# hedgepigdaniel/video-annotator

Measured on AMD Instinct MI355X. Metric: stabilized frames/sec at 4K NV12, 1/2/4/8 GPU; remap % HBM roofline, higher is better.
Workload: dtype u8 pixels / f32 map / f64 rotations

## Files before the change

video-annotator_amd/csrc/vstab_track.hip:

```cpp
#include <algorithm>
#include <climits>

#include <hip/hip_ext.h>

#include "vstab_internal.hpp"
#include "vstab_track.hpp"

namespace vstab {

__device__ __forceinline__ int reflect101(int i, int n) {
    if (n == 1) return 0;
    while (i < 0 || i >= n) i = i < 0 ? -i : 2 * n - 2 - i;
    return i;
}

__device__ __forceinline__ uint32_t load4_reflect_row(const uint8_t *__restrict__ row, int w, int gx, bool vec_ok) {
    if (vec_ok && gx >= 0 && gx + 4 <= w) return *reinterpret_cast<const uint32_t *>(row + gx);
    uint32_t v = 0;
#pragma unroll
    for (int i = 0; i < 4; i++) v |= (uint32_t)row[reflect101(gx + i, w)] << (8 * i);
    return v;
}

__device__ __forceinline__ uint32_t load4_reflect(const uint8_t *__restrict__ src, uint32_t pitch, int w, int h, int gx,
// ... 51 lines not shown
                d[j][0] = p[0], d[j][1] = p[1], d[j][2] = p[2], d[j][3] = p[3];
            }
        }
    } else {
#pragma unroll
        for (int q = 0; q < 4; q++) {
            const int gx = sx0 + 4 * q;
            if (vec_ok && gx >= 0 && gx + 4 <= sw) {
#pragma unroll
                for (int j = 0; j < 5; j++) d[j][q] = *reinterpret_cast<const uint32_t *>(row[j] + gx);
            } else {
                int col[4];
#pragma unroll
                for (int i = 0; i < 4; i++) col[i] = NEAR ? min(abs(gx + i), 2 * sw - 2 - abs(gx + i)) : reflect101(gx + i, sw);
#pragma unroll
                for (int j = 0; j < 5; j++)
                    d[j][q] = (uint32_t)row[j][col[0]] | ((uint32_t)row[j][col[1]] << 8) | ((uint32_t)row[j][col[2]] << 16) | ((uint32_t)row[j][col[3]] << 24);
            }
        }
    }
    if (COPY) {
#pragma unroll
        for (int jj = 2; jj <= 3; jj++) {
            const int r = 2 * y + jj - 2;
            if (r >= sh) break;
            uint8_t *o = cp + (uint32_t)r * cpitch + (uint32_t)(2 * x0);
            if (!EDGE) {
                *reinterpret_cast<uint2 *>(o) = make_uint2(d[jj][1], d[jj][2]);
            } else {
#pragma unroll
                for (int b = 0; b < 8; b++)
                    if (2 * x0 + b < sw) o[b] = (uint8_t)((b < 4 ? d[jj][1] : d[jj][2]) >> (8 * (b & 3)));
            }
        }
    }
    return pyr_down_dot4x4(d);
}

template <bool EDGE, bool NEAR, bool COPY = false>
__device__ __forceinline__ void pyr_down_group(const uint8_t *__restrict__ src, uint32_t spitch, int sw, int sh, uint8_t *__restrict__ dst, size_t dpitch,
                                               int dw, int x0, int y, bool vec_ok, uint8_t *__restrict__ cp = nullptr, uint32_t cpitch = 0) {
    const uint32_t out = pyr_down_group4<EDGE, NEAR, COPY>(src, spitch, sw, sh, x0, y, vec_ok, cp, cpitch);
    uint8_t *o = dst + (size_t)((uint32_t)y * (uint32_t)dpitch) + x0;
    if (!EDGE) {
        *reinterpret_cast<uint32_t *>(o) = out;
    } else {
        for (int c = 0; c < 4 && x0 + c < dw; c++) o[c] = (uint8_t)(out >> (8 * c));
    }
}

__global__ void __launch_bounds__(256) k_pyr_down(const uint8_t *__restrict__ src, size_t spitch, int sw, int sh,
                                                  uint8_t *__restrict__ dst, size_t dpitch, int dw, int dh, int vec_ok, int g_lo, int g_hi,
                                                  int nbx, int nb_edge, int n_groups, int near) {
    if ((int)blockIdx.x >= nb_edge) {
        const int b = blockIdx.x - nb_edge, by = b / nbx, bx = b - by * nbx;
        const int g = g_lo + bx * 64 + (threadIdx.x & 63), y = by * 4 + (threadIdx.x >> 6);
        if (g >= g_hi || y >= dh) return;
        pyr_down_group<false, true>(src, (uint32_t)spitch, sw, sh, dst, dpitch, dw, 4 * g, y, true);
    } else {
        const int n_edge = n_groups - (g_hi - g_lo);
        const int e = blockIdx.x * 256 + threadIdx.x;
        const int y = e / n_edge, i = e - y * n_edge;
        if (y >= dh) return;
        const int g = i < g_lo ? i : g_hi + (i - g_lo);
        if (near)
            pyr_down_group<true, true>(src, (uint32_t)spitch, sw, sh, dst, dpitch, dw, 4 * g, y, vec_ok != 0);
        else
            pyr_down_group<true, false>(src, (uint32_t)spitch, sw, sh, dst, dpitch, dw, 4 * g, y, vec_ok != 0);
    }
}

__global__ void __launch_bounds__(256) k_pack_pyr(const uint8_t *__restrict__ src, uint32_t spitch, int sw, int sh, uint8_t *__restrict__ dst, uint32_t dpitch,
                                                  int dw, int dh, int vec_ok, int g_lo, int g_hi, int nbx, int nb_edge, int n_groups, int near, int nb_pyr,
                                                  const uint8_t *__restrict__ uv, uint32_t uvpitch, uint8_t *__restrict__ ring, uint32_t rpitch, int uv_vec) {
    if ((int)blockIdx.x >= nb_pyr) {
        uint8_t *cdst = ring + (uint32_t)sh * rpitch;
        const int rows = sh / 2;
        if (uv_vec) {
            const int vecs = sw / 16;
            for (int e = ((int)blockIdx.x - nb_pyr) * 256 + threadIdx.x; e < rows * vecs; e += ((int)gridDim.x - nb_pyr) * 256) {
                const int r = e / vecs, c = e - r * vecs;
                reinterpret_cast<uint4 *>(cdst + (uint32_t)r * rpitch)[c] = reinterpret_cast<const uint4 *>(uv + (uint32_t)r * uvpitch)[c];
            }
        } else {
            for (int e = ((int)blockIdx.x - nb_pyr) * 256 + threadIdx.x; e < rows * sw; e += ((int)gridDim.x - nb_pyr) * 256) {
                const int r = e / sw, c = e - r * sw;
                cdst[(uint32_t)r * rpitch + c] = uv[(uint32_t)r * uvpitch + c];
            }
        }
        return;
    }
    if ((int)blockIdx.x >= nb_edge) {
        const int b = blockIdx.x - nb_edge, by = b / nbx, bx = b - by * nbx;
        const int g = g_lo + bx * 64 + (threadIdx.x & 63), y = by * 4 + (threadIdx.x >> 6);
        if (g >= g_hi || y >= dh) return;
        pyr_down_group<false, true, true>(src, spitch, sw, sh, dst, dpitch, dw, 4 * g, y, true, ring, rpitch);
    } else {
        const int n_edge = n_groups - (g_hi - g_lo);
        const int e = blockIdx.x * 256 + threadIdx.x;
        const int y = e / n_edge, i = e - y * n_edge;
        if (y >= dh) return;
        const int g = i < g_lo ? i : g_hi + (i - g_lo);
        if (near)
            pyr_down_group<true, true, true>(src, spitch, sw, sh, dst, dpitch, dw, 4 * g, y, vec_ok != 0, ring, rpitch);
        else
            pyr_down_group<true, false, true>(src, spitch, sw, sh, dst, dpitch, dw, 4 * g, y, vec_ok != 0, ring, rpitch);
    }
}

constexpr int P2_TW = 16, P2_TH = 10;
constexpr int P2_MG = (2 * P2_TW + 5 + 3) / 4, P2_MW = 4 * P2_MG;
constexpr int P2_MH = 2 * P2_TH + 3;
constexpr int P2_ITEMS = P2_MG * P2_MH, P2_ROUNDS = (P2_ITEMS + 255) / 256;
static_assert(P2_TW % 4 == 0 && 2 * P2_TW + 5 <= P2_MW, "the region holds the taps of the tile's last output");

template <bool NEAR>
__device__ __forceinline__ void pyr_down_x2_tile(const uint8_t *__restrict__ src, uint32_t spitch, int sw, int sh, uint8_t *__restrict__ mid, uint32_t mpitch, int mw,
                                                 int mh, uint8_t *__restrict__ dst, uint32_t dpitch, int dw, int dh, bool vec_ok, bool dst_vec_ok,
                                                 uint8_t (&smid)[P2_MH][P2_MW]) {
    const int tid = threadIdx.x;
    const int x0 = blockIdx.x * P2_TW, y0 = blockIdx.y * P2_TH;
    const int mx0 = 2 * x0 - 4, my0 = 2 * y0 - 2;
    const bool interior = vec_ok && mx0 >= 2 && my0 >= 1 && mx0 + P2_MW <= mw && my0 + P2_MH <= mh && 2 * (mx0 + P2_MW) + 4 <= sw && 2 * (my0 + P2_MH) + 1 <= sh;
    if (interior) {
        uint32_t d[P2_ROUNDS][5][4];
#pragma unroll
        for (int k = 0; k < P2_ROUNDS; k++) {
            const int it = min(tid + 256 * k, P2_ITEMS - 1);
            const int ry = it / P2_MG, g = it - ry * P2_MG;
            const uint8_t *r0 = src + (uint32_t)(2 * (my0 + ry) - 2) * spitch + (uint32_t)(2 * (mx0 + 4 * g) - 4);
#pragma unroll
            for (int j = 0; j < 5; j++) {
                const uint4 v = *reinterpret_cast<const uint4 *>(r0 + (uint32_t)j * spitch);
                d[k][j][0] = v.x, d[k][j][1] = v.y, d[k][j][2] = v.z, d[k][j][3] = v.w;
            }
        }
#pragma unroll
        for (int k = 0; k < P2_ROUNDS; k++) {
            const int it = tid + 256 * k;
            if (it >= P2_ITEMS) break;
            const int ry = it / P2_MG, g = it - ry * P2_MG;
            const uint32_t out = pyr_down_dot4x4(d[k]);
            *reinterpret_cast<uint32_t *>(&smid[ry][4 * g]) = out;
            if (g >= 1 && g <= P2_TW / 2 && ry >= 2 && ry < 2 + 2 * P2_TH) *reinterpret_cast<uint32_t *>(mid + (uint32_t)(my0 + ry) * mpitch + (mx0 + 4 * g)) = out;
        }
    } else {
#pragma unroll 1
        for (int k = 0; k < P2_ROUNDS; k++) {
            const int it = tid + 256 * k;
            if (it >= P2_ITEMS) break;
            const int ry = it / P2_MG, g = it - ry * P2_MG;
            const int my = my0 + ry, mx = mx0 + 4 * g;
            if (my < 0 || my >= mh || mx < 0 || mx >= mw) continue;
            const uint32_t out = pyr_down_group4<true, NEAR>(src, spitch, sw, sh, mx, my, vec_ok);
            *reinterpret_cast<uint32_t *>(&smid[ry][4 * g]) = out;
            if (g >= 1 && g <= P2_TW / 2 && ry >= 2 && ry < 2 + 2 * P2_TH) {
                uint8_t *o = mid + (uint32_t)my * mpitch + mx;
                if (vec_ok && mx + 4 <= mw) *reinterpret_cast<uint32_t *>(o) = out;
                else
                    for (int c = 0; c < 4 && mx + c < mw; c++) o[c] = (uint8_t)(out >> (8 * c));
            }
        }
    }
    __syncthreads();
    if (interior) {
        if (tid < (P2_TW / 4) * P2_TH) {
            const int ty = tid / (P2_TW / 4), g = tid - ty * (P2_TW / 4);
            uint32_t d[5][4];
#pragma unroll
            for (int j = 0; j < 5; j++) {
                const uint2 lo = *reinterpret_cast<const uint2 *>(&smid[2 * ty + j][8 * g]), hi = *reinterpret_cast<const uint2 *>(&smid[2 * ty + j][8 * g + 8]);
                d[j][0] = lo.x, d[j][1] = lo.y, d[j][2] = hi.x, d[j][3] = hi.y;
            }
            const uint32_t out = pyr_down_dot4x4(d);
            uint8_t *o = dst + (uint32_t)(y0 + ty) * dpitch + (x0 + 4 * g);
            if (dst_vec_ok) *reinterpret_cast<uint32_t *>(o) = out;
            else
                for (int c = 0; c < 4; c++) o[c] = (uint8_t)(out >> (8 * c));
        }
    } else {
        for (int e = tid; e < P2_TW * P2_TH; e += 256) {
            const int ty = e / P2_TW, tx = e - ty * P2_TW;
            const int x = x0 + tx, y = y0 + ty;
            if (x >= dw || y >= dh) continue;
            int col[5];
#pragma unroll
            for (int i = 0; i < 5; i++) col[i] = reflect101(2 * x - 2 + i, mw) - mx0;
            uint32_t acc = 128u;
#pragma unroll
            for (int j = 0; j < 5; j++) {
                const uint8_t *r = smid[reflect101(2 * y - 2 + j, mh) - my0];
                const uint32_t k = j == 0 || j == 4 ? 1u : j == 2 ? 6u : 4u;
                acc += k * ((uint32_t)r[col[0]] + 4u * r[col[1]] + 6u * r[col[2]] + 4u * r[col[3]] + r[col[4]]);
            }
            dst[(uint32_t)y * dpitch + x] = (uint8_t)(acc >> 8);
        }
    }
}

__global__ void __launch_bounds__(256) k_pyr_down_x2(const uint8_t *__restrict__ src, uint32_t spitch, int sw, int sh, uint8_t *__restrict__ mid,
                                                     uint32_t mpitch, int mw, int mh, uint8_t *__restrict__ dst, uint32_t dpitch, int dw, int dh, int vec_ok,
                                                     int dst_vec_ok, int near) {
    __shared__ __attribute__((aligned(16))) uint8_t smid[P2_MH][P2_MW];
    if (near) pyr_down_x2_tile<true>(src, spitch, sw, sh, mid, mpitch, mw, mh, dst, dpitch, dw, dh, vec_ok != 0, dst_vec_ok != 0, smid);
    else pyr_down_x2_tile<false>(src, spitch, sw, sh, mid, mpitch, mw, mh, dst, dpitch, dw, dh, vec_ok != 0, dst_vec_ok != 0, smid);
}

constexpr int ME_TW = 64, ME_TH = 16, ME_SW = ME_TW + 8, ME_SH = ME_TH + 4;

__global__ void __launch_bounds__(256) k_min_eig(const uint8_t *__restrict__ src, size_t pitch, int w, int h,
                                                 float *__restrict__ eig, int *__restrict__ max_bits, int vec_ok) {
    __shared__ __attribute__((aligned(16))) uint8_t tile[ME_SH][ME_SW];
    __shared__ float dxs[ME_TH + 2][ME_TW + 2 + 1], dys[ME_TH + 2][ME_TW + 2 + 1];
    __shared__ int bmax;
    const int tid = threadIdx.x;
    const int ox = blockIdx.x * ME_TW, oy = blockIdx.y * ME_TH;
    const int sx0 = ox - 4, sy0 = oy - 2;
    if (tid == 0) bmax = INT_MIN;
    for (int e = tid; e < ME_SH * (ME_SW / 4); e += 256) {
        const int ry = e / (ME_SW / 4), rd = e - ry * (ME_SW / 4);
        reinterpret_cast<uint32_t *>(&tile[ry][0])[rd] = load4_reflect(src, (uint32_t)pitch, w, h, sx0 + 4 * rd, sy0 + ry, vec_ok != 0);
    }
    __syncthreads();
    const float scale = (float)(1.0 / (4.0 * 3.0 * 255.0));
    const float k0 = 2.0f * scale, k1 = scale;
    for (int e = tid; e < (ME_TH + 2) * (ME_TW + 2); e += 256) {
        const int ry = e / (ME_TW + 2), rx = e - ry * (ME_TW + 2);
        const uint8_t *c = &tile[ry + 1][rx + 3];
        const int a00 = c[-ME_SW - 1], a01 = c[-ME_SW], a02 = c[-ME_SW + 1];
        const int a10 = c[-1], a12 = c[1];
        const int a20 = c[ME_SW - 1], a21 = c[ME_SW], a22 = c[ME_SW + 1];
        const float d0 = (float)(a02 - a00), d1 = (float)(a12 - a10), d2 = (float)(a22 - a20);
        float dx = (d0 + d2) * k1 + d1 * k0;
        const float s0 = (float)a01 * k0 + ((float)a00 + (float)a02) * k1;
        const float s2 = (float)a21 * k0 + ((float)a20 + (float)a22) * k1;
        float dy = s2 - s0;
        const int gx = ox - 1 + rx, gy = oy - 1 + ry;
        if (gx < 0 || gx >= w) dx = -dx;
        if (gy < 0 || gy >= h) dy = -dy;
        dxs[ry][rx] = dx, dys[ry][rx] = dy;
    }
    __syncthreads();
    const int q = tid & 15, ty = tid >> 4;
    const int x = ox + 4 * q, y = oy + ty;
    int best = INT_MIN;
    if (x < w && y < h) {
        float a_[3][6], b_[3][6];
#pragma unroll
        for (int j = 0; j < 3; j++)
#pragma unroll
            for (int i = 0; i < 6; i++) a_[j][i] = dxs[ty + j][4 * q + i], b_[j][i] = dys[ty + j][4 * q + i];
        float ev[4];
#pragma unroll
        for (int c = 0; c < 4; c++) {
            double sxx = 0, sxy = 0, syy = 0;
#pragma unroll
            for (int j = 0; j < 3; j++)
#pragma unroll
                for (int i = 0; i < 3; i++) {
                    const float a = a_[j][c + i], b = b_[j][c + i];
                    sxx += (double)(a * a), sxy += (double)(a * b), syy += (double)(b * b);
                }
            const float a = (float)sxx * 0.5f, b = (float)sxy, cc = (float)syy * 0.5f;
            ev[c] = (a + cc) - sqrtf((a - cc) * (a - cc) + b * b);
            if (x + c < w) best = max(best, __float_as_int(ev[c]));
        }
        float *o = eig + (size_t)y * w + x;
        if (vec_ok && (w & 3) == 0 && x + 4 <= w) {
            *reinterpret_cast<float4 *>(o) = make_float4(ev[0], ev[1], ev[2], ev[3]);
        } else {
            for (int c = 0; c < 4 && x + c < w; c++) o[c] = ev[c];
        }
    }
    best = max(best, __builtin_amdgcn_update_dpp(INT_MIN, best, 0x111, 0xf, 0xf, false));
    best = max(best, __builtin_amdgcn_update_dpp(INT_MIN, best, 0x112, 0xf, 0xf, false));
    best = max(best, __builtin_amdgcn_update_dpp(INT_MIN, best, 0x114, 0xf, 0xf, false));
    best = max(best, __builtin_amdgcn_update_dpp(INT_MIN, best, 0x118, 0xf, 0xf, false));
    if (q == 15) atomicMax(&bmax, best);
    __syncthreads();
    if (tid == 0) atomicMax(max_bits, bmax);
}

__global__ void __launch_bounds__(256) k_corner_candidates(const float *__restrict__ eig, int w, int h,
                                                           const int *__restrict__ max_bits, double quality,
                                                           unsigned long long *__restrict__ keys,
                                                           unsigned int *__restrict__ count, unsigned int cap) {
    const int x = blockIdx.x * 64 + threadIdx.x, y = blockIdx.y * 4 + threadIdx.y;
    if (x < 1 || y < 1 || x >= w - 1 || y >= h - 1) return;
    const float thr = (float)((double)__int_as_float(*max_bits) * quality);
    const float *p = eig + (size_t)y * w + x;
    const float v = p[0];
    if (!(v > thr)) return;
    float m = v;
    m = fmaxf(m, p[-w - 1]), m = fmaxf(m, p[-w]), m = fmaxf(m, p[-w + 1]);
    m = fmaxf(m, p[-1]), m = fmaxf(m, p[1]);
    m = fmaxf(m, p[w - 1]), m = fmaxf(m, p[w]), m = fmaxf(m, p[w + 1]);
    if (v != m) return;
    const unsigned int slot = atomicAdd(count, 1u);
    if (slot < cap) keys[slot] = ((unsigned long long)__float_as_uint(v) << 32) | (unsigned int)(y * w + x);
}

constexpr int CF_TW = 64, CF_TH = 31;
constexpr int CF_EH = CF_TH + 2;
constexpr int CF_DH = 36, CF_DP = 68;
constexpr int CF_SW = 72, CF_SH = 38;
constexpr int CF_EP = 67;
constexpr int CF_SLOTS = 256;

__device__ __forceinline__ float ubyte_f32(uint32_t v, int b) { return (float)((v >> (8 * b)) & 255u); }

template <bool DENSE>
__device__ __forceinline__ void cf_nonmax(const float (&es)[CF_EH][CF_EP], int tid, int ox, int oy, int w, int h, float thr_lb,
                                          unsigned long long *__restrict__ my_slots, unsigned int *bcount, float *__restrict__ dense) {
    const int tx = tid & 63, r0 = (tid >> 6) * 8;
    const int x = ox + tx;
    float rm0 = fmaxf(fmaxf(es[r0][tx], es[r0][tx + 1]), es[r0][tx + 2]);
    float c1 = es[r0 + 1][tx + 1];
    float rm1 = fmaxf(fmaxf(es[r0 + 1][tx], c1), es[r0 + 1][tx + 2]);
#pragma unroll
    for (int r = 0; r < 8; r++) {
        const int ty = r0 + r;
        if (ty >= CF_TH) break;
        const float c2 = es[ty + 2][tx + 1];
        const float rm2 = fmaxf(fmaxf(es[ty + 2][tx], c2), es[ty + 2][tx + 2]);
        const float m = fmaxf(fmaxf(rm0, rm1), rm2);
        const int y = oy + ty;
        const bool cand = x >= 1 && y >= 1 && x < w - 1 && y < h - 1 && c1 > thr_lb && c1 == m;
        if (DENSE) {
            dense[ty * CF_TW + tx] = cand ? c1 : -__builtin_inff();
        } else {
            const unsigned long long ballot = __ballot(cand);
            if (ballot) {
                unsigned int base = 0;
                if (tx == 0) base = atomicAdd(bcount, (unsigned int)__popcll(ballot));
                base = __builtin_amdgcn_readfirstlane(base);
                const unsigned int slot = base + __builtin_amdgcn_mbcnt_hi((uint32_t)(ballot >> 32), __builtin_amdgcn_mbcnt_lo((uint32_t)ballot, 0));
                if (cand && slot < CF_SLOTS) my_slots[slot] = ((unsigned long long)__float_as_uint(c1) << 32) | (unsigned int)(y * w + x);
            }
        }
        rm0 = rm1, rm1 = rm2, c1 = c2;
    }
}

__global__ void __launch_bounds__(256) k_corners_fused(const uint8_t *__restrict__ src, size_t pitch, int w, int h, double quality,
                                                       unsigned int *__restrict__ max_key, unsigned long long *__restrict__ slots,
                                                       unsigned int *__restrict__ tile_counts, float *__restrict__ spill, int vec_ok) {
    __shared__ __attribute__((aligned(16))) uint8_t tile[CF_SH][CF_SW];
    __shared__ __attribute__((aligned(16))) float dxs[CF_DH][CF_DP], dys[CF_DH][CF_DP];
    __shared__ float es[CF_EH][CF_EP];
    __shared__ int bmax;
    __shared__ unsigned int bcount;
    const int tid = threadIdx.x;
    const int ox = blockIdx.x * CF_TW, oy = blockIdx.y * CF_TH;
    const unsigned int seen = __hip_atomic_load(max_key, __ATOMIC_RELAXED, __HIP_MEMORY_SCOPE_AGENT);
    if (tid == 0) bmax = INT_MIN, bcount = 0;
    for (int e = tid; e < CF_SH * (CF_SW / 4); e += 256) {
        const int ry = e / (CF_SW / 4), rd = e - ry * (CF_SW / 4);
        reinterpret_cast<uint32_t *>(&tile[ry][0])[rd] = load4_reflect(src, (uint32_t)pitch, w, h, ox - 4 + 4 * rd, oy - 3 + ry, vec_ok != 0);
    }
    __syncthreads();
    const float scale = (float)(1.0 / (4.0 * 3.0 * 255.0));
    const float k0 = 2.0f * scale, k1 = scale;
    if (tid < 17 * 12) {
        const int g = tid / 17, c = tid - g * 17;
        float D[5][4], S[5][4];
#pragma unroll
        for (int j = 0; j < 5; j++) {
            const uint32_t *row = reinterpret_cast<const uint32_t *>(&tile[3 * g + j][4 * c]);
            const uint32_t lo = row[0], hi = row[1];
            const float f[6] = {ubyte_f32(lo, 1), ubyte_f32(lo, 2), ubyte_f32(lo, 3), ubyte_f32(hi, 0), ubyte_f32(hi, 1), ubyte_f32(hi, 2)};
#pragma unroll
            for (int i = 0; i < 4; i++) {
                D[j][i] = f[i + 2] - f[i];
                S[j][i] = f[i + 1] * k0 + (f[i] + f[i + 2]) * k1;
            }
        }
#pragma unroll
        for (int r = 0; r < 3; r++) {
            const int gy = oy - 2 + 3 * g + r;
            const bool fy = gy < 0 || gy >= h;
            float dx[4], dy[4];
#pragma unroll
            for (int i = 0; i < 4; i++) {
                const int gx = ox - 2 + 4 * c + i;
                dx[i] = (D[r][i] + D[r + 2][i]) * k1 + D[r + 1][i] * k0;
                dy[i] = S[r + 2][i] - S[r][i];
                if (gx < 0 || gx >= w) dx[i] = -dx[i];
                if (fy) dy[i] = -dy[i];
            }
            *reinterpret_cast<float4 *>(&dxs[3 * g + r][4 * c]) = make_float4(dx[0], dx[1], dx[2], dx[3]);
            *reinterpret_cast<float4 *>(&dys[3 * g + r][4 * c]) = make_float4(dy[0], dy[1], dy[2], dy[3]);
        }
    }
    __syncthreads();
    int best = INT_MIN;
    if (tid < 22 * 11) {
        const int by = tid / 22, bx = tid - by * 22;
        float a_[5][5], b_[5][5];
#pragma unroll
        for (int j = 0; j < 5; j++)
#pragma unroll
            for (int i = 0; i < 5; i++) a_[j][i] = dxs[3 * by + j][3 * bx + i], b_[j][i] = dys[3 * by + j][3 * bx + i];
        float sum[3][3][3];
#pragma unroll
        for (int q = 0; q < 3; q++) {
            double col[3][5];
#pragma unroll
            for (int j = 0; j < 5; j++)
#pragma unroll
                for (int i = 0; i < 5; i++) {
                    const float u = q == 2 ? b_[j][i] : a_[j][i], v = q == 0 ? a_[j][i] : b_[j][i];
                    const double p = (double)(u * v);
#pragma unroll
                    for (int e = 0; e < 3; e++)
                        if (j >= e && j <= e + 2) col[e][i] = j == e ? p : col[e][i] + p;
                }
#pragma unroll
            for (int e = 0; e < 3; e++)
#pragma unroll
                for (int i = 0; i < 3; i++) sum[q][e][i] = (float)((col[e][i] + col[e][i + 1]) + col[e][i + 2]);
        }
#pragma unroll
        for (int e = 0; e < 3; e++)
#pragma unroll
            for (int i = 0; i < 3; i++) {
                const float a = sum[0][e][i] * 0.5f, b = sum[1][e][i], cc = sum[2][e][i] * 0.5f;
                const float ev = (a + cc) - sqrtf((a - cc) * (a - cc) + b * b);
                es[3 * by + e][3 * bx + i] = ev;
                const int gx = ox - 1 + 3 * bx + i, gy = oy - 1 + 3 * by + e;
                if (gx >= 0 && gx < w && gy >= 0 && gy < h) best = max(best, __float_as_int(ev));
            }
    }
    best = max(best, __builtin_amdgcn_update_dpp(INT_MIN, best, 0x111, 0xf, 0xf, false));
    best = max(best, __builtin_amdgcn_update_dpp(INT_MIN, best, 0x112, 0xf, 0xf, false));
    best = max(best, __builtin_amdgcn_update_dpp(INT_MIN, best, 0x114, 0xf, 0xf, false));
    best = max(best, __builtin_amdgcn_update_dpp(INT_MIN, best, 0x118, 0xf, 0xf, false));
    best = max(best, __builtin_amdgcn_update_dpp(INT_MIN, best, 0x142, 0xa, 0xf, false));
    best = max(best, __builtin_amdgcn_update_dpp(INT_MIN, best, 0x143, 0xc, 0xf, false));
    if ((tid & 63) == 63) atomicMax(&bmax, best);
    __syncthreads();
    const int tile_max = bmax;
    if (tid == 0 && ((unsigned int)tile_max ^ 0x80000000u) > seen) atomicMax(max_key, (unsigned int)tile_max ^ 0x80000000u);
    const int lb_bits = max(tile_max, (int)(seen ^ 0x80000000u));
    const float thr_lb = lb_bits >= 0 ? (float)((double)__int_as_float(lb_bits) * quality) : -__builtin_inff();
    const int tile_idx = blockIdx.y * gridDim.x + blockIdx.x;
    cf_nonmax<false>(es, tid, ox, oy, w, h, thr_lb, slots + (size_t)tile_idx * CF_SLOTS, &bcount, nullptr);
    __syncthreads();
    const unsigned int n = bcount;
    if (tid == 0) tile_counts[tile_idx] = n;
    if (n > CF_SLOTS) cf_nonmax<true>(es, tid, ox, oy, w, h, thr_lb, nullptr, nullptr, spill + (size_t)tile_idx * (CF_TW * CF_TH));
}

constexpr int FK_TILES = 16;
__global__ void __launch_bounds__(256) k_filter_keys(const unsigned long long *__restrict__ slots, const unsigned int *__restrict__ tile_counts,
                                                     const float *__restrict__ spill, int n_tiles, int tiles_x, int w,
                                                     const unsigned int *__restrict__ max_key, double quality,
                                                     unsigned long long *__restrict__ out, unsigned int *__restrict__ counts, unsigned int cap_out) {
    __shared__ unsigned long long kept[FK_TILES * CF_SLOTS];
    __shared__ unsigned int n_kept, base, n_spilled;
    const int tid = threadIdx.x, wave = tid >> 6, lane = tid & 63;
    if (tid == 0) n_kept = 0, n_spilled = 0;
    __syncthreads();
    const float thr = (float)((double)__int_as_float((int)(*max_key ^ 0x80000000u)) * quality);
    for (int k = 0; k < FK_TILES / 4; k++) {
        const int t = blockIdx.x * FK_TILES + wave * (FK_TILES / 4) + k;
        if (t >= n_tiles) break;
        const unsigned int n = tile_counts[t];
        if (n > CF_SLOTS) {
            if (lane == 0) atomicAdd(&n_spilled, 1u);
            const int ty0 = t / tiles_x, ox = (t - ty0 * tiles_x) * CF_TW, oy = ty0 * CF_TH;
            float v[CF_TH];
#pragma unroll
            for (int r = 0; r < CF_TH; r++) v[r] = spill[(size_t)t * (CF_TW * CF_TH) + r * CF_TW + lane];
#pragma unroll
            for (int r = 0; r < CF_TH; r++) {
                const bool keep = v[r] > thr;
                const unsigned long long ballot = __ballot(keep);
                if (ballot) {
                    unsigned int b = 0;
                    if (lane == 0) b = atomicAdd(&counts[0], (unsigned int)__popcll(ballot));
                    b = __builtin_amdgcn_readfirstlane(b);
                    const unsigned int slot = b + __builtin_amdgcn_mbcnt_hi((uint32_t)(ballot >> 32), __builtin_amdgcn_mbcnt_lo((uint32_t)ballot, 0));
                    if (keep && slot < cap_out) out[slot] = ((unsigned long long)__float_as_uint(v[r]) << 32) | (unsigned int)((oy + r) * w + ox + lane);
                }
            }
            continue;
        }
        for (unsigned int i = lane; i < ((n + 63) & ~63u); i += 64) {
            unsigned long long key = 0;
            bool keep = false;
            if (i < n) {
                key = slots[(size_t)t * CF_SLOTS + i];
                keep = __uint_as_float((unsigned int)(key >> 32)) > thr;
            }
            const unsigned long long ballot = __ballot(keep);
            if (ballot) {
                unsigned int b = 0;
                if (lane == 0) b = atomicAdd(&n_kept, (unsigned int)__popcll(ballot));
                b = __builtin_amdgcn_readfirstlane(b);
                if (keep) kept[b + __builtin_amdgcn_mbcnt_hi((uint32_t)(ballot >> 32), __builtin_amdgcn_mbcnt_lo((uint32_t)ballot, 0))] = key;
            }
        }
    }
    __syncthreads();
    const unsigned int n = n_kept;
    if (tid == 0) {
        if (n) base = atomicAdd(&counts[0], n);
        if (n_spilled) atomicAdd(&counts[1], n_spilled);
    }
    __syncthreads();
    for (unsigned int i = tid; i < n; i += 256)
        if (base + i < cap_out) out[base + i] = kept[i];
}

constexpr int LKW = 21, LKR = 24, LKT = 22;
constexpr int LKJM = 5, LKJR = LKT + 2 * LKJM;

__device__ __forceinline__ int wave_sum_i32(int v) {
    v += __builtin_amdgcn_update_dpp(0, v, 0x111, 0xf, 0xf, false);
    v += __builtin_amdgcn_update_dpp(0, v, 0x112, 0xf, 0xf, false);
    v += __builtin_amdgcn_update_dpp(0, v, 0x114, 0xf, 0xf, false);
    v += __builtin_amdgcn_update_dpp(0, v, 0x118, 0xf, 0xf, false);
    v += __builtin_amdgcn_update_dpp(0, v, 0x142, 0xa, 0xf, false);
    v += __builtin_amdgcn_update_dpp(0, v, 0x143, 0xc, 0xf, false);
    return __builtin_amdgcn_readlane(v, 63);
}
#define LK_DESCALE(x, n) (((x) + (1 << ((n)-1))) >> (n))
__device__ __forceinline__ float lk_level_scale(int l) { return __uint_as_float((uint32_t)(127 - l) << 23); }
__device__ __forceinline__ int lk_mul(int a, int b) { return __mul24(a, b); }
__device__ __forceinline__ int lk_mad(int a, int b, int c) {
    int d;
    asm("v_mad_i32_i24 %0, %1, %2, %3" : "=v"(d) : "v"(a), "v"(b), "v"(c));
    return d;
}
constexpr bool lk_div_magic_ok(int d, int magic) {
    for (int e = 0; e < 600; e++)
        if (((e * magic) >> 16) != e / d) return false;
    return true;
}
static_assert(lk_div_magic_ok(22, 2979) && lk_div_magic_ok(21, 3121), "division constants");
__device__ __forceinline__ int lk_div22(int e) { return __mul24(e, 2979) >> 16; }
__device__ __forceinline__ int lk_div21(int k) { return __mul24(k, 3121) >> 16; }

constexpr int LK_THREADS = 256, LK_WAVES = 4;
#ifndef VSTAB_LK_PRIO
#define VSTAB_LK_PRIO 1
#endif
constexpr int LK_WPAD = (LKW * LKW + 63) & ~63;

__device__ __forceinline__ void lk_level_matrix(float s0, float s1, float s2, float *out) {
    const float FLT_SCALE = 1.0f / (1 << 20);
    const float A11 = s0 * FLT_SCALE, A12 = s1 * FLT_SCALE, A22 = s2 * FLT_SCALE;
    const float D = A11 * A22 - A12 * A12;
    const float minEig = ((A22 + A11) - sqrtf((A11 - A22) * (A11 - A22) + (4.f * A12) * A12)) / (float)(2 * LKW * LKW);
    out[0] = A11, out[1] = A12, out[2] = A22, out[3] = 1.f / D;
    out[4] = minEig < 1e-4f || D < 1.1920928955078125e-7f ? 1.0f : 0.0f;
}

template <int N>
__device__ __forceinline__ void wave_sums_i32(int (&t)[N]) {
#define VSTAB_DPP_STEP(ctrl, rows)                                                          \
    _Pragma("unroll") for (int i = 0; i < N; i++) t[i] += __builtin_amdgcn_update_dpp(0, t[i], ctrl, rows, 0xf, false)
    VSTAB_DPP_STEP(0x111, 0xf);
    VSTAB_DPP_STEP(0x112, 0xf);
    VSTAB_DPP_STEP(0x114, 0xf);
    VSTAB_DPP_STEP(0x118, 0xf);
    VSTAB_DPP_STEP(0x142, 0xa);
    VSTAB_DPP_STEP(0x143, 0xc);
#undef VSTAB_DPP_STEP
#pragma unroll
    for (int i = 0; i < N; i++) t[i] = __builtin_amdgcn_readlane(t[i], 63);
}

template <int SIDE, int THREADS = LK_THREADS>
struct LkStage {
    static_assert(SIDE % 4 == 0, "rows are split into dwords");
    static constexpr int ROWW = SIDE / 4, NW = SIDE * ROWW, N = (NW + THREADS - 1) / THREADS;
    uint32_t v[N];
    __device__ __forceinline__ void load(const uint8_t *img, uint32_t pitch, int w, int h, int x0, int y0, int tid) {
        const bool interior = x0 >= 0 && y0 >= 0 && x0 + SIDE <= w && y0 + SIDE <= h;
#pragma unroll
        for (int k = 0; k < N; k++) {
            const int e = tid + THREADS * k;
            v[k] = 0;
            if (e < NW) {
                const int ry = e / ROWW, rx = 4 * (e - ry * ROWW);
                if (interior) {
                    __builtin_memcpy(&v[k], img + __umul24((uint32_t)(y0 + ry), pitch) + (uint32_t)(x0 + rx), 4);
                } else {
                    const uint8_t *row = img + __umul24((uint32_t)reflect101(y0 + ry, h), pitch);
                    v[k] = (uint32_t)row[reflect101(x0 + rx, w)] | ((uint32_t)row[reflect101(x0 + rx + 1, w)] << 8) |
                           ((uint32_t)row[reflect101(x0 + rx + 2, w)] << 16) | ((uint32_t)row[reflect101(x0 + rx + 3, w)] << 24);
                }
            }
        }
    }
    __device__ __forceinline__ void load_interior(const uint8_t *img, uint32_t pitch, int x0, int y0, int tid) {
#pragma unroll
        for (int k = 0; k < N; k++) {
            const int e = min(tid + THREADS * k, NW - 1);
            const int ry = e / ROWW, rx = 4 * (e - ry * ROWW);
            __builtin_memcpy(&v[k], img + __umul24((uint32_t)(y0 + ry), pitch) + (uint32_t)(x0 + rx), 4);
        }
    }
    template <int OUT>
    __device__ __forceinline__ void store_window(int *dst, int tid, int dx, int dy) const {
#pragma unroll
        for (int k = 0; k < N; k++) {
            const int e = tid + THREADS * k;
            const int ry = e / ROWW, rx = 4 * (e - ry * ROWW);
            const int Y = ry - dy, X = rx - dx;
            if (e < NW && (unsigned)Y < (unsigned)OUT) {
                int *o = dst + lk_mul(Y, OUT) + X;
#pragma unroll
                for (int i = 0; i < 4; i++)
                    if ((unsigned)(X + i) < (unsigned)OUT) o[i] = (int)((v[k] >> (8 * i)) & 255u);
            }
        }
    }
    __device__ __forceinline__ void store(int *dst, int tid) const {
#pragma unroll
        for (int k = 0; k < N; k++) {
            const int e = tid + THREADS * k;
            if (e < NW) *reinterpret_cast<int4 *>(dst + 4 * e) = make_int4((int)(v[k] & 255u), (int)((v[k] >> 8) & 255u), (int)((v[k] >> 16) & 255u), (int)(v[k] >> 24));
        }
    }
};

__device__ __forceinline__ uint4 make_record(float x, float y, unsigned int status, unsigned int seq) {
    return make_uint4(__float_as_uint(x), seq, __float_as_uint(y), (seq << 2) | status);
}
__device__ __forceinline__ unsigned int record_status(const uint4 &r) { return r.w & 3u; }

#ifdef VSTAB_DEV
__device__ unsigned long long *g_lk_timing = nullptr;
extern "C" __attribute__((visibility("default"))) void vstab_dev_set_lk_timing(void *p) {
    (void)hipMemcpyToSymbol(HIP_SYMBOL(g_lk_timing), &p, sizeof(p));
}
#define LK_STAMP(k, v) \
    if (g_lk_timing && tid == 0) g_lk_timing[(((size_t)(seq & 63u) * 256 + (size_t)f) << 5) + (k)] = (v)
#define LK_STAMP1(k, v) \
    if (g_lk_timing && tid == 64) g_lk_timing[(((size_t)(seq & 63u) * 256 + (size_t)f) << 5) + (k)] = (v)
#define LK_NOW() __builtin_amdgcn_s_memrealtime()
#else
#define LK_STAMP(k, v)
#define LK_STAMP1(k, v)
#define LK_NOW() 0ull
#endif

__global__ void __launch_bounds__(LK_THREADS, 3) k_lk_track(LkSegArgs args) {
    __shared__ __attribute__((aligned(16))) int regI[LK_MAX_LEVELS][LKR * LKR];
    __shared__ uint32_t dpk[LK_MAX_LEVELS][LKT * LKT];
    __shared__ short patch_i[LK_MAX_LEVELS][LK_WPAD];
    __shared__ uint32_t patch_xy[LK_MAX_LEVELS][LK_WPAD];
    __shared__ float level_mat[LK_MAX_LEVELS][8];
    __shared__ __attribute__((aligned(16))) int regJ[2][LKJR * LKJR];
    const int f = blockIdx.x, tid = threadIdx.x, lane = tid & 63, wave = __builtin_amdgcn_readfirstlane(tid >> 6);
    const int n = args.n;
    if (f >= n) return;
    unsigned long long *const clk = args.clk;
    __builtin_amdgcn_s_setprio(VSTAB_LK_PRIO);
    if (clk && tid == 0) atomicMin(&clk[0], wall_clock64());
    unsigned int seq = args.seq[0];
    LK_STAMP(0, LK_NOW());
    float2 pp;
    if (args.chain_in) {
        const uint4 r = args.chain_in[f];
        const bool tagged = r.y == args.parent_seq && (r.w >> 2) == (args.parent_seq & 0x3fffffffu);
        if (!tagged || record_status(r) != 1u) {
            if (tid == 0) {
                for (int i = 0; i < args.n_frames; i++) {
                    const uint4 dead = make_record(0.0f, 0.0f, tagged && record_status(r) != 3u ? 2u : 3u, args.seq[i]);
                    if (args.dev_rec[i]) args.dev_rec[i][f] = dead;
                    if (args.host_rec[i]) args.host_rec[i][f] = dead;
                }
            }
            return;
        }
        pp = make_float2(__uint_as_float(r.x), __uint_as_float(r.z));
    } else {
        pp = args.prev_pts[f];
    }
    const float half = (LKW - 1) * 0.5f;
    constexpr int LK_PPL = (LKW * LKW + 63) / 64;
    int koff[LK_PPL];
#pragma unroll
    for (int m = 0; m < LK_PPL; m++) {
        const int k = lane + 64 * m;
        const int wy = lk_div21(k), wx = k - lk_mul(wy, LKW);
        koff[m] = k < LKW * LKW ? lk_mul(wy, LKJR) + wx : 0;
    }
    __shared__ float s_result[4];
    __shared__ float s_est[2][2];
    LkStage<LKJR, LK_THREADS - 64> pfIt, pfJt;
    LkStage<LKJR, 64> pfIo;
    constexpr int PF_NONE = INT_MIN / 2;
    constexpr int PF_SLACK = (LKJR - LKR) / 2;
    __shared__ int s_pf[LK_MAX_LEVELS][4];
    __shared__ int s_jorg[2][2];
#pragma unroll 1
    for (int fi = 0; fi < args.n_frames; fi++) {
    const LkPyramid &I = args.pyr[fi], &J = args.pyr[fi + 1];
    seq = args.seq[fi];
    if (fi) LK_STAMP(0, LK_NOW());
    LK_STAMP(1, LK_NOW());
    float2 np = make_float2(0.f, 0.f);
    int st = 1;
    const int max_level = I.levels - 1;
    int jb = 0;
    int jorg_x = PF_NONE, jorg_y = PF_NONE;
    int own_dx = -1, own_dy = -1;
    {
        LkStage<LKR> si[LK_MAX_LEVELS];
        LkStage<LKJR> sj;
        bool iok[LK_MAX_LEVELS];
        int top_dx = -1, top_dy = -1;
        bool top_ahead = false;
#pragma unroll
        for (int l = 0; l < LK_MAX_LEVELS; l++) {
            iok[l] = false;
            if (l > max_level) continue;
            int ax = PF_NONE, ay = PF_NONE;
            if (fi) ax = __builtin_amdgcn_readfirstlane(s_pf[l][0]), ay = __builtin_amdgcn_readfirstlane(s_pf[l][1]);
            const float lscale = lk_level_scale(l);
            const int ipx = (int)floorf(pp.x * lscale - half), ipy = (int)floorf(pp.y * lscale - half);
            if (ipx < -LKW || ipx >= I.w[l] || ipy < -LKW || ipy >= I.h[l]) continue;
            const int dx = ipx - 1 - ax, dy = ipy - 1 - ay;
            if ((unsigned)dx <= (unsigned)(2 * PF_SLACK) && (unsigned)dy <= (unsigned)(2 * PF_SLACK)) {
                if (l == max_level) top_dx = dx, top_dy = dy;
                else if (l == max_level - wave) own_dx = dx, own_dy = dy;
            } else {
                iok[l] = true;
                si[l].load(I.img[l], (uint32_t)I.pitch[l], I.w[l], I.h[l], ipx - 1, ipy - 1, tid);
            }
            if (l == max_level) {
                int bx = PF_NONE, by = PF_NONE;
                if (fi) bx = __builtin_amdgcn_readfirstlane(s_pf[l][2]), by = __builtin_amdgcn_readfirstlane(s_pf[l][3]);
                if (ipx - 2 >= bx && ipy - 2 >= by && ipx + LKT + 2 <= bx + LKJR && ipy + LKT + 2 <= by + LKJR) {
                    jorg_x = bx, jorg_y = by, top_ahead = true;
                } else {
                    jorg_x = ipx - LKJM, jorg_y = ipy - LKJM;
                    sj.load(J.img[l], (uint32_t)J.pitch[l], I.w[l], I.h[l], jorg_x, jorg_y, tid);
                }
            }
        }
#pragma unroll
        for (int l = 0; l < LK_MAX_LEVELS; l++)
            if (iok[l]) si[l].store(regI[l], tid);
        if (top_ahead && wave != 0) pfJt.store(regJ[0], tid - 64);
        if (top_dx >= 0 && wave != 0) pfIt.template store_window<LKR>(regI[max_level], tid - 64, top_dx, top_dy);
        if (jorg_x != PF_NONE && !top_ahead) sj.store(regJ[0], tid);
        LK_STAMP(17, (unsigned long long)((top_dx >= 0 ? 1 : 0) | (top_ahead ? 2 : 0)));
    }
// ... 385 lines not shown
```

Baseline: 27830.

## Restructure fused corner kernel: shared structure-tensor products, interior fast path, batched atomics

The fused Shi-Tomasi corner kernel now computes the dx*dx, dx*dy and dy*dy products once per pixel into shared memory, instead of each 3x3 box thread recomputing them from stored gradients. Boundary sign flips are applied to the cross product, and the eigenvalue array reuses the products buffer. A templated interior path skips reflect-border checks and uses plain vector loads for tiles away from the image edge. Non-max suppression now issues one LDS atomicAdd per wave instead of one per row, and division by constants uses magic multiplies with the ubyte-to-float conversion done in inline asm. Shared memory grows from two planes to three, which may lower occupancy, and an extra barrier separates the eigen reads from the es writes that alias prod.

```diff
diff --git a/video-annotator_amd/csrc/vstab_track.hip b/video-annotator_amd/csrc/vstab_track.hip
--- a/video-annotator_amd/csrc/vstab_track.hip
+++ b/video-annotator_amd/csrc/vstab_track.hip
@@ -377,124 +377,176 @@
 
 constexpr int CF_TW = 64, CF_TH = 31;
 constexpr int CF_EH = CF_TH + 2;
-constexpr int CF_DH = 36, CF_DP = 68;
+constexpr int CF_DH = 35, CF_DP = 68;
 constexpr int CF_SW = 72, CF_SH = 38;
 constexpr int CF_EP = 67;
 constexpr int CF_SLOTS = 256;
-
-__device__ __forceinline__ float ubyte_f32(uint32_t v, int b) { return (float)((v >> (8 * b)) & 255u); }
-
-template <bool DENSE>
+constexpr int CF_PC = CF_DP / 4, CF_PR = 5, CF_PG = CF_DH / CF_PR;
+constexpr int CF_BX = 22, CF_BY = 11;
+static_assert(CF_PC * 4 == CF_DP && CF_PG * CF_PR == CF_DH && CF_DH + 2 <= CF_SH && CF_PC * CF_PG <= 256, "prod ownership covers the region");
+static_assert(CF_BX * 3 == CF_TW + 2 && CF_BY * 3 == CF_EH && CF_EH + 2 == CF_DH && CF_BX * CF_BY <= 256, "box ownership covers the region");
+static_assert(CF_EH * CF_EP <= CF_DH * CF_DP, "the eigenvalues fit the plane they take over");
+
+constexpr bool cf_div_magic_ok(int d, int magic, int n) {
+    for (int e = 0; e < n; e++)
+        if (((e * magic) >> 16) != e / d) return false;
+    return true;
+}
+static_assert(cf_div_magic_ok(CF_SW / 4, 3641, CF_SH * (CF_SW / 4) + 256) && cf_div_magic_ok(CF_PC, 3856, 256) && cf_div_magic_ok(CF_BX, 2979, 256),
+              "division constants");
+
+template <int B>
+__device__ __forceinline__ float ubyte_f32(uint32_t v) {
+    float f;
+    if (B == 0) asm("v_cvt_f32_ubyte0 %0, %1" : "=v"(f) : "v"(v));
+    if (B == 1) asm("v_cvt_f32_ubyte1 %0, %1" : "=v"(f) : "v"(v));
+    if (B == 2) asm("v_cvt_f32_ubyte2 %0, %1" : "=v"(f) : "v"(v));
+    if (B == 3) asm("v_cvt_f32_ubyte3 %0, %1" : "=v"(f) : "v"(v));
+    return f;
+}
+
+template <bool DENSE, bool INTERIOR>
 __device__ __forceinline__ void cf_nonmax(const float (&es)[CF_EH][CF_EP], int tid, int ox, int oy, int w, int h, float thr_lb,
                                           unsigned long long *__restrict__ my_slots, unsigned int *bcount, float *__restrict__ dense) {
-    const int tx = tid & 63, r0 = (tid >> 6) * 8;
+    const int tx = tid & 63, r0 = __builtin_amdgcn_readfirstlane(tid >> 6) * 8;
     const int x = ox + tx;
+    const bool x_in = INTERIOR || (x >= 1 && x < w - 1);
     float rm0 = fmaxf(fmaxf(es[r0][tx], es[r0][tx + 1]), es[r0][tx + 2]);
     float c1 = es[r0 + 1][tx + 1];
     float rm1 = fmaxf(fmaxf(es[r0 + 1][tx], c1), es[r0 + 1][tx + 2]);
+    float v[8];
+    bool cand[8];
+    unsigned long long ballot[8];
+    unsigned int total = 0;
 #pragma unroll
     for (int r = 0; r < 8; r++) {
         const int ty = r0 + r;
-        if (ty >= CF_TH) break;
-        const float c2 = es[ty + 2][tx + 1];
-        const float rm2 = fmaxf(fmaxf(es[ty + 2][tx], c2), es[ty + 2][tx + 2]);
+        const bool row = r < 7 || ty < CF_TH;
+        const int below = r < 7 ? ty + 2 : min(ty + 2, CF_EH - 1);
+        const float c2 = es[below][tx + 1];
+        const float rm2 = fmaxf(fmaxf(es[below][tx], c2), es[below][tx + 2]);
         const float m = fmaxf(fmaxf(rm0, rm1), rm2);
         const int y = oy + ty;
-        const bool cand = x >= 1 && y >= 1 && x < w - 1 && y < h - 1 && c1 > thr_lb && c1 == m;
+        cand[r] = row && x_in && (INTERIOR || (y >= 1 && y < h - 1)) && c1 > thr_lb && c1 == m;
         if (DENSE) {
-            dense[ty * CF_TW + tx] = cand ? c1 : -__builtin_inff();
+            if (row) dense[ty * CF_TW + tx] = cand[r] ? c1 : -__builtin_inff();
         } else {
-            const unsigned long long ballot = __ballot(cand);
-            if (ballot) {
-                unsigned int base = 0;
-                if (tx == 0) base = atomicAdd(bcount, (unsigned int)__popcll(ballot));
-                base = __builtin_amdgcn_readfirstlane(base);
-                const unsigned int slot = base + __builtin_amdgcn_mbcnt_hi((uint32_t)(ballot >> 32), __builtin_amdgcn_mbcnt_lo((uint32_t)ballot, 0));
-                if (cand && slot < CF_SLOTS) my_slots[slot] = ((unsigned long long)__float_as_uint(c1) << 32) | (unsigned int)(y * w + x);
-            }
+            v[r] = c1;
+            ballot[r] = __builtin_amdgcn_ballot_w64(cand[r]);
+            total += (unsigned int)__popcll(ballot[r]);
         }
         rm0 = rm1, rm1 = rm2, c1 = c2;
     }
-}
-
-__global__ void __launch_bounds__(256) k_corners_fused(const uint8_t *__restrict__ src, size_t pitch, int w, int h, double quality,
-                                                       unsigned int *__restrict__ max_key, unsigned long long *__restrict__ slots,
-                                                       unsigned int *__restrict__ tile_counts, float *__restrict__ spill, int vec_ok) {
-    __shared__ __attribute__((aligned(16))) uint8_t tile[CF_SH][CF_SW];
-    __shared__ __attribute__((aligned(16))) float dxs[CF_DH][CF_DP], dys[CF_DH][CF_DP];
-    __shared__ float es[CF_EH][CF_EP];
-    __shared__ int bmax;
-    __shared__ unsigned int bcount;
-    const int tid = threadIdx.x;
-    const int ox = blockIdx.x * CF_TW, oy = blockIdx.y * CF_TH;
-    const unsigned int seen = __hip_atomic_load(max_key, __ATOMIC_RELAXED, __HIP_MEMORY_SCOPE_AGENT);
-    if (tid == 0) bmax = INT_MIN, bcount = 0;
-    for (int e = tid; e < CF_SH * (CF_SW / 4); e += 256) {
-        const int ry = e / (CF_SW / 4), rd = e - ry * (CF_SW / 4);
-        reinterpret_cast<uint32_t *>(&tile[ry][0])[rd] = load4_reflect(src, (uint32_t)pitch, w, h, ox - 4 + 4 * rd, oy - 3 + ry, vec_ok != 0);
-    }
-    __syncthreads();
+    if (!DENSE && total) {
+        unsigned int base = 0;
+        if (tx == 0) base = atomicAdd(bcount, total);
+        base = __builtin_amdgcn_readfirstlane(base);
+#pragma unroll
+        for (int r = 0; r < 8; r++) {
+            if (!ballot[r]) continue;
+            const unsigned int slot = base + __builtin_amdgcn_mbcnt_hi((uint32_t)(ballot[r] >> 32), __builtin_amdgcn_mbcnt_lo((uint32_t)ballot[r], 0));
+            if (cand[r] && slot < CF_SLOTS) my_slots[slot] = ((unsigned long long)__float_as_uint(v[r]) << 32) | (unsigned int)((oy + r0 + r) * w + x);
+            base += (unsigned int)__popcll(ballot[r]);
+        }
+    }
+}
+
+constexpr int CF_LOADS = (CF_SH * (CF_SW / 4) + 255) / 256;
+template <bool INTERIOR>
+__device__ __forceinline__ void cf_load(uint32_t (&v)[CF_LOADS], const uint8_t *__restrict__ src, uint32_t pitch, int w, int h, int ox, int oy, bool vec_ok,
+                                        int tid) {
+#pragma unroll
+    for (int k = 0; k < CF_LOADS; k++) {
+        const int e = tid + 256 * k;
+        const int ry = __mul24(e, 3641) >> 16, rd = e - ry * (CF_SW / 4);
+        v[k] = 0;
+        if (e >= CF_SH * (CF_SW / 4)) continue;
+        if (INTERIOR) v[k] = *reinterpret_cast<const uint32_t *>(src + ((uint32_t)(oy - 3 + ry) * pitch + (uint32_t)(ox - 4 + 4 * rd)));
+        else v[k] = load4_reflect(src, pitch, w, h, ox - 4 + 4 * rd, oy - 3 + ry, vec_ok);
+    }
+}
+__device__ __forceinline__ void cf_store(uint8_t (&tile)[CF_SH][CF_SW], const uint32_t (&v)[CF_LOADS], int tid) {
+#pragma unroll
+    for (int k = 0; k < CF_LOADS; k++)
+        if (tid + 256 * k < CF_SH * (CF_SW / 4)) reinterpret_cast<uint32_t *>(&tile[0][0])[tid + 256 * k] = v[k];
+}
+
+template <bool INTERIOR>
+__device__ __forceinline__ void cf_products(const uint8_t (&tile)[CF_SH][CF_SW], float (&prod)[3][CF_DH][CF_DP], int ox, int oy, int w, int h, int tid) {
+    if (tid >= CF_PC * CF_PG) return;
     const float scale = (float)(1.0 / (4.0 * 3.0 * 255.0));
     const float k0 = 2.0f * scale, k1 = scale;
-    if (tid < 17 * 12) {
-        const int g = tid / 17, c = tid - g * 17;
-        float D[5][4], S[5][4];
-#pragma unroll
-        for (int j = 0; j < 5; j++) {
-            const uint32_t *row = reinterpret_cast<const uint32_t *>(&tile[3 * g + j][4 * c]);
-            const uint32_t lo = row[0], hi = row[1];
-            const float f[6] = {ubyte_f32(lo, 1), ubyte_f32(lo, 2), ubyte_f32(lo, 3), ubyte_f32(hi, 0), ubyte_f32(hi, 1), ubyte_f32(hi, 2)};
-#pragma unroll
-            for (int i = 0; i < 4; i++) {
-                D[j][i] = f[i + 2] - f[i];
-                S[j][i] = f[i + 1] * k0 + (f[i] + f[i + 2]) * k1;
-            }
-        }
-#pragma unroll
-        for (int r = 0; r < 3; r++) {
-            const int gy = oy - 2 + 3 * g + r;
-            const bool fy = gy < 0 || gy >= h;
-            float dx[4], dy[4];
-#pragma unroll
-            for (int i = 0; i < 4; i++) {
-                const int gx = ox - 2 + 4 * c + i;
-                dx[i] = (D[r][i] + D[r + 2][i]) * k1 + D[r + 1][i] * k0;
-                dy[i] = S[r + 2][i] - S[r][i];
-                if (gx < 0 || gx >= w) dx[i] = -dx[i];
-                if (fy) dy[i] = -dy[i];
-            }
-            *reinterpret_cast<float4 *>(&dxs[3 * g + r][4 * c]) = make_float4(dx[0], dx[1], dx[2], dx[3]);
-            *reinterpret_cast<float4 *>(&dys[3 * g + r][4 * c]) = make_float4(dy[0], dy[1], dy[2], dy[3]);
+    const int g = __mul24(tid, 3856) >> 16, c = tid - g * CF_PC;
+    uint32_t flip_x[4];
+#pragma unroll
+    for (int i = 0; i < 4; i++) {
+        const int gx = ox - 2 + 4 * c + i;
+        flip_x[i] = !INTERIOR && (gx < 0 || gx >= w) ? 0x80000000u : 0u;
+    }
+    float D[CF_PR + 2][4], S[CF_PR + 2][4];
+#pragma unroll
+    for (int j = 0; j < CF_PR + 2; j++) {
+        const uint32_t *row = reinterpret_cast<const uint32_t *>(&tile[CF_PR * g + j][4 * c]);
+        const uint32_t lo = row[0], hi = row[1];
+        const float f[6] = {ubyte_f32<1>(lo), ubyte_f32<2>(lo), ubyte_f32<3>(lo), ubyte_f32<0>(hi), ubyte_f32<1>(hi), ubyte_f32<2>(hi)};
+#pragma unroll
+        for (int i = 0; i < 4; i++) {
+            D[j][i] = f[i + 2] - f[i];
+            S[j][i] = f[i + 1] * k0 + (f[i] + f[i + 2]) * k1;
+        }
+    }
+#pragma unroll
+    for (int r = 0; r < CF_PR; r++) {
+        const int gy = oy - 2 + CF_PR * g + r;
+        const uint32_t flip_y = !INTERIOR && (gy < 0 || gy >= h) ? 0x80000000u : 0u;
+        float xx[4], xy[4], yy[4];
+#pragma unroll
+        for (int i = 0; i < 4; i++) {
+            const float dx = (D[r][i] + D[r + 2][i]) * k1 + D[r + 1][i] * k0;
+            const float dy = S[r + 2][i] - S[r][i];
+            xx[i] = dx * dx, yy[i] = dy * dy;
+            xy[i] = INTERIOR ? dx * dy : __uint_as_float(__float_as_uint(dx * dy) ^ flip_x[i] ^ flip_y);
+        }
+        *reinterpret_cast<float4 *>(&prod[0][CF_PR * g + r][4 * c]) = make_float4(xx[0], xx[1], xx[2], xx[3]);
+        *reinterpret_cast<float4 *>(&prod[1][CF_PR * g + r][4 * c]) = make_float4(xy[0], xy[1], xy[2], xy[3]);
+        *reinterpret_cast<float4 *>(&prod[2][CF_PR * g + r][4 * c]) = make_float4(yy[0], yy[1], yy[2], yy[3]);
+    }
+}
+
+__device__ __forceinline__ void cf_sum3of5(double p0, double p1, double p2, double p3, double p4, double &s0, double &s1, double &s2) {
+    const double m = p1 + p2;
+    s0 = p0 + m, s1 = m + p3, s2 = (p2 + p3) + p4;
+}
+
+template <bool INTERIOR>
+__device__ __forceinline__ int cf_eigenvalues(const float (&prod)[3][CF_DH][CF_DP], float (&es)[CF_EH][CF_EP], int ox, int oy, int w, int h, int tid) {
+    const bool active = tid < CF_BX * CF_BY;
+    const int t = min(tid, CF_BX * CF_BY - 1);
+    const int by = __mul24(t, 2979) >> 16, bx = t - by * CF_BX;
+    float sum[3][3][3];
+    {
+#pragma unroll
+        for (int q = 0; q < 3; q++) {
+            double col[3][5];
+#pragma unroll
+            for (int i = 0; i < 5; i++) {
+                double p[5];
+#pragma unroll
+                for (int j = 0; j < 5; j++) p[j] = (double)prod[q][3 * by + j][3 * bx + i];
+                cf_sum3of5(p[0], p[1], p[2], p[3], p[4], col[0][i], col[1][i], col[2][i]);
+            }
+#pragma unroll
+            for (int e = 0; e < 3; e++) {
+                double s[3];
+                cf_sum3of5(col[e][0], col[e][1], col[e][2], col[e][3], col[e][4], s[0], s[1], s[2]);
+#pragma unroll
+                for (int i = 0; i < 3; i++) sum[q][e][i] = (float)s[i];
+            }
         }
     }
     __syncthreads();
     int best = INT_MIN;
-    if (tid < 22 * 11) {
-        const int by = tid / 22, bx = tid - by * 22;
-        float a_[5][5], b_[5][5];
-#pragma unroll
-        for (int j = 0; j < 5; j++)
-#pragma unroll
-            for (int i = 0; i < 5; i++) a_[j][i] = dxs[3 * by + j][3 * bx + i], b_[j][i] = dys[3 * by + j][3 * bx + i];
-        float sum[3][3][3];
-#pragma unroll
-        for (int q = 0; q < 3; q++) {
-            double col[3][5];
-#pragma unroll
-            for (int j = 0; j < 5; j++)
-#pragma unroll
-                for (int i = 0; i < 5; i++) {
-                    const float u = q == 2 ? b_[j][i] : a_[j][i], v = q == 0 ? a_[j][i] : b_[j][i];
-                    const double p = (double)(u * v);
-#pragma unroll
-                    for (int e = 0; e < 3; e++)
-                        if (j >= e && j <= e + 2) col[e][i] = j == e ? p : col[e][i] + p;
-                }
-#pragma unroll
-            for (int e = 0; e < 3; e++)
-#pragma unroll
-                for (int i = 0; i < 3; i++) sum[q][e][i] = (float)((col[e][i] + col[e][i + 1]) + col[e][i + 2]);
-        }
+    if (active) {
 #pragma unroll
         for (int e = 0; e < 3; e++)
 #pragma unroll
@@ -503,9 +555,29 @@
                 const float ev = (a + cc) - sqrtf((a - cc) * (a - cc) + b * b);
                 es[3 * by + e][3 * bx + i] = ev;
                 const int gx = ox - 1 + 3 * bx + i, gy = oy - 1 + 3 * by + e;
-                if (gx >= 0 && gx < w && gy >= 0 && gy < h) best = max(best, __float_as_int(ev));
-            }
-    }
+                if (INTERIOR || (gx >= 0 && gx < w && gy >= 0 && gy < h)) best = max(best, __float_as_int(ev));
+            }
+    }
+    return best;
+}
+
+template <bool INTERIOR>
+__device__ __forceinline__ void cf_tile(uint8_t (&tile)[CF_SH][CF_SW], float (&prod)[3][CF_DH][CF_DP], int &bmax, unsigned int &bcount, unsigned int &bseen,
+                                        const uint8_t *__restrict__ src, uint32_t pitch, int w, int h, double quality, unsigned int *__restrict__ max_key,
+                                        unsigned long long *__restrict__ slots, unsigned int *__restrict__ tile_counts, float *__restrict__ spill, bool vec_ok) {
+    float (&es)[CF_EH][CF_EP] = *reinterpret_cast<float (*)[CF_EH][CF_EP]>(&prod[0][0][0]);
+    const int tid = threadIdx.x;
+    const int ox = blockIdx.x * CF_TW, oy = blockIdx.y * CF_TH;
+    uint32_t v[CF_LOADS];
+    cf_load<INTERIOR>(v, src, pitch, w, h, ox, oy, vec_ok, tid);
+    if (tid == 0) bmax = INT_MIN, bcount = 0;
+    cf_store(tile, v, tid);
+    unsigned int seen = 0;
+    if (tid == 255) seen = __hip_atomic_load(max_key, __ATOMIC_RELAXED, __HIP_MEMORY_SCOPE_AGENT);
+    __syncthreads();
+    cf_products<INTERIOR>(tile, prod, ox, oy, w, h, tid);
+    __syncthreads();
+    int best = cf_eigenvalues<INTERIOR>(prod, es, ox, oy, w, h, tid);
     best = max(best, __builtin_amdgcn_update_dpp(INT_MIN, best, 0x111, 0xf, 0xf, false));
     best = max(best, __builtin_amdgcn_update_dpp(INT_MIN, best, 0x112, 0xf, 0xf, false));
     best = max(best, __builtin_amdgcn_update_dpp(INT_MIN, best, 0x114, 0xf, 0xf, false));
@@ -513,17 +585,36 @@
     best = max(best, __builtin_amdgcn_update_dpp(INT_MIN, best, 0x142, 0xa, 0xf, false));
     best = max(best, __builtin_amdgcn_update_dpp(INT_MIN, best, 0x143, 0xc, 0xf, false));
     if ((tid & 63) == 63) atomicMax(&bmax, best);
+    if (tid == 255) bseen = seen;
     __syncthreads();
     const int tile_max = bmax;
+    seen = bseen;
     if (tid == 0 && ((unsigned int)tile_max ^ 0x80000000u) > seen) atomicMax(max_key, (unsigned int)tile_max ^ 0x80000000u);
     const int lb_bits = max(tile_max, (int)(seen ^ 0x80000000u));
     const float thr_lb = lb_bits >= 0 ? (float)((double)__int_as_float(lb_bits) * quality) : -__builtin_inff();
     const int tile_idx = blockIdx.y * gridDim.x + blockIdx.x;
-    cf_nonmax<false>(es, tid, ox, oy, w, h, thr_lb, slots + (size_t)tile_idx * CF_SLOTS, &bcount, nullptr);
+    cf_nonmax<false, INTERIOR>(es, tid, ox, oy, w, h, thr_lb, slots + (size_t)tile_idx * CF_SLOTS, &bcount, nullptr);
     __syncthreads();
     const unsigned int n = bcount;
     if (tid == 0) tile_counts[tile_idx] = n;
-    if (n > CF_SLOTS) cf_nonmax<true>(es, tid, ox, oy, w, h, thr_lb, nullptr, nullptr, spill + (size_t)tile_idx * (CF_TW * CF_TH));
+    if (n > CF_SLOTS) cf_nonmax<true, INTERIOR>(es, tid, ox, oy, w, h, thr_lb, nullptr, nullptr, spill + (size_t)tile_idx * (CF_TW * CF_TH));
+}
+
+__device__ __forceinline__ bool cf_interior(int ox, int oy, int w, int h, int vec_ok) {
+    return vec_ok && ox >= 4 && ox - 4 + CF_SW <= w && oy >= 3 && oy - 3 + CF_SH <= h;
+}
+
+__global__ void __launch_bounds__(256) k_corners_fused(const uint8_t *__restrict__ src, size_t pitch, int w, int h, double quality,
+                                                       unsigned int *__restrict__ max_key, unsigned long long *__restrict__ slots,
+                                                       unsigned int *__restrict__ tile_counts, float *__restrict__ spill, int vec_ok) {
+    __shared__ __attribute__((aligned(16))) uint8_t tile[CF_SH][CF_SW];
+    __shared__ __attribute__((aligned(16))) float prod[3][CF_DH][CF_DP];
+    __shared__ int bmax;
+    __shared__ unsigned int bcount, bseen;
+    if (cf_interior(blockIdx.x * CF_TW, blockIdx.y * CF_TH, w, h, vec_ok))
+        cf_tile<true>(tile, prod, bmax, bcount, bseen, src, (uint32_t)pitch, w, h, quality, max_key, slots, tile_counts, spill, true);
+    else
+        cf_tile<false>(tile, prod, bmax, bcount, bseen, src, (uint32_t)pitch, w, h, quality, max_key, slots, tile_counts, spill, vec_ok != 0);
 }
 
 constexpr int FK_TILES = 16;
```

After: 28210 (median of 6 runs). 1.01x the previous value.
